# marcopesavento/Super-resolution-3D-Human-Shape-from-a-Single-Low-Resolution-Image

Measured on AMD Instinct MI355X. Metric: occupancy queries/sec (dense 512^3 reconstruction: encoder + query sweep + 2x marching cubes), higher is better.
Workload: dtype bf16

## Files before the change

super-resolution-3d-human-shape-from-a-single-low-resolution-image_amd/csrc/surs_api.cpp:

```cpp
#include "surs_common.h"

extern "C" int surs_abi_version(void) { return SURS_ABI_VERSION; }

extern "C" const char *surs_last_error(void) { return surs::err_buf(); }

extern "C" int surs_device_info(int *cu_count, char *arch_out) {
    int dev = 0;
    SURS_HIP_CHECK(hipGetDevice(&dev));
    hipDeviceProp_t prop;
    SURS_HIP_CHECK(hipGetDeviceProperties(&prop, dev));
    if (cu_count) *cu_count = prop.multiProcessorCount;
    if (arch_out) {
        strncpy(arch_out, prop.gcnArchName, 31);
        arch_out[31] = 0;
    }
    return 0;
}

#include <atomic>
#include <cstdlib>
#include <mutex>

namespace {
struct OptionRow {
    const char *name, *env;
    int def;
    char env_first;
    int env_value;
    const char *what;
};
const OptionRow kOptions[surs::OPT_COUNT] = {
    {"split_parts", "SURS_SPLIT", 2, 'b', 3, "operand parts of the fp32-grade GEMMs: 2 (f16 x 2) or 3 (bf16 x 3; env: bf16x3)"},
    {"grid_f32_columns", "SURS_GRID_F32", 1, 'g', 0, "0 (env: gemm): the fp32 sweep on the per-point layer kernels"},
    {"grid_kernel", "SURS_GRID_KERNEL", 0, 0, 0, "reduced-precision column kernel: 0 (default 12), 3, 10, 12"},
    {"grid_f32_kernel", "SURS_GRID_F32_KERNEL", 0, 0, 0, "fp32-grade column kernel: 0 (default 11), 5, 11"},
    {"r_parts", "SURS_R_PARTS", 1, 0, 0, "1: the bf16 sweep's R vectors from one f16 part; 0: the sweep's split"},
    {"grid_f32_passes", "SURS_GRID_F32_PASSES", 2, 0, 0, "passes of the fp32-grade column kernel per batch: 2 (lr, then hr) or 1"},
    {"bicubic_block", "SURS_BICUBIC_BLOCK", 1, 0, 0, "0: bicubic x2 with statistics one output per item (A/B; same bits)"},
    {"mc_emit_reclassify", "SURS_MC_EMIT_RECLASSIFY", 0, 0, 0, "1: marching cubes' emit pass classifies again (tests)"},
    {"point_runs_speculate", "SURS_POINT_RUNS_SPECULATE", 1, 0, 0, "0: surs_query_points_columns reads the run count before it launches"},
    {"conv_trace", "SURS_CONV_TRACE", 0, 0, 0, "diagnostic builds (-DSURS_CONV_TRACE): print the 3x3 kernel's phase stamps"},
    {"v3_trace", "SURS_V3_TRACE", 0, 0, 0, "diagnostic builds (-DSURS_V3_TRACE): print the column kernels' stamps"},
    {"conv_tall_min_wg", "SURS_CONV_TALL_MIN_WG", 256, 0, 0, "workgroups from which a stride-1 3x3 convolution takes the 8-row tile instead of 4 rows (0: never; same bits)"},
    {"conv_wide_min_wg", "SURS_CONV_WIDE_MIN_WG", 512, 0, 0, "workgroups (of 64 channels) from which such a launch takes 8 rows x 64 channels (part of the bits: another order of sums; 0: never)"},
    {"mc_ring", "SURS_MC_RING", 258, 0, 0, "planes of marching cubes' edge -> vertex-id ring = layers per chunk of a one-piece extraction + 1 (66: round 5's)"},
    {"rvec_small", "SURS_RVEC_SMALL", 1, 0, 0, "0: the affine part's GEMM of batches of <= 1024 columns on the 256 x 256-tile kernel (A/B; same bits)"},
    {"r_fused", "SURS_R_FUSED", 1, 0, 0, "0: the bf16 sweep's R vectors of batches of > 1024 columns from the g-scaled image and two GEMM launches (A/B; same bits)"},
};
std::atomic<int> g_option[surs::OPT_COUNT];
std::once_flag g_option_once;
void import_environment() {
    for (int i = 0; i < surs::OPT_COUNT; ++i) {
        const OptionRow &r = kOptions[i];
        int v = r.def;
        if (const char *e = getenv(r.env)) {
            if (r.env_first) v = (e[0] == r.env_first) ? r.env_value : r.def;
            else if (e[0]) v = atoi(e);
        }
        g_option[i].store(v, std::memory_order_relaxed);
    }
}
int find_option(const char *name) {
    if (!name) return -1;
    for (int i = 0; i < surs::OPT_COUNT; ++i)
        if (!strcmp(name, kOptions[i].name) || !strcmp(name, kOptions[i].env)) return i;
    return -1;
}
}

int surs::option(surs::Opt id) {
    std::call_once(g_option_once, import_environment);
    return g_option[id].load(std::memory_order_relaxed);
}

extern "C" int surs_set_option(const char *name, int value) {
    const int i = find_option(name);
    SURS_REQUIRE(i >= 0, "unknown option '%s' (surs_option_name(i) lists them)", name ? name : "(null)");
    std::call_once(g_option_once, import_environment);
    g_option[i].store(value, std::memory_order_relaxed);
    return 0;
// ... 12 lines not shown
```

super-resolution-3d-human-shape-from-a-single-low-resolution-image_amd/csrc/surs_common.h:

```cpp
#pragma once
#include <hip/hip_runtime.h>

#include <cstdarg>
#include <cstdio>
#include <cstring>

#include "../../include/surs.h"

namespace surs {

inline char *err_buf() {
    static thread_local char buf[512] = "";
    return buf;
}

inline int fail(int code, const char *fmt, ...) {
    va_list ap;
    va_start(ap, fmt);
    vsnprintf(err_buf(), 512, fmt, ap);
    va_end(ap);
    return code;
}

#define SURS_HIP_CHECK(expr)                                                                     \
    do {                                                                                         \
        hipError_t e_ = (expr);                                                                  \
        if (e_ != hipSuccess)                                                                    \
            return surs::fail(SURS_E_HIP, "%s:%d %s -> %s", __FILE__, __LINE__, #expr, hipGetErrorString(e_)); \
    } while (0)

#define SURS_LAUNCH_CHECK() SURS_HIP_CHECK(hipGetLastError())

#define SURS_REQUIRE(cond, ...)                                   \
    do {                                                          \
        if (!(cond)) return surs::fail(SURS_E_INVALID, __VA_ARGS__); \
    } while (0)

#ifndef SURS_ABL_NO_ISA_PINS
#define SURS_ISA_PIN(v) asm volatile("" : "+v"(v))
#else
#define SURS_ISA_PIN(v) do { } while (0)
#endif

enum Opt {
    OPT_SPLIT_PARTS, OPT_GRID_F32_COLUMNS, OPT_GRID_KERNEL, OPT_GRID_F32_KERNEL, OPT_R_PARTS,
    OPT_GRID_F32_PASSES, OPT_BICUBIC_BLOCK, OPT_MC_EMIT_RECLASSIFY, OPT_POINT_RUNS_SPECULATE, OPT_CONV_TRACE,
    OPT_V3_TRACE, OPT_CONV_TALL_MIN_WG, OPT_CONV_WIDE_MIN_WG, OPT_MC_RING, OPT_RVEC_SMALL, OPT_R_FUSED, OPT_COUNT
};
int option(Opt id);

inline hipStream_t as_stream(void *s) { return reinterpret_cast<hipStream_t>(s); }

constexpr int ceil_div(long long a, long long b) { return (int)((a + b - 1) / b); }

struct DeviceOnce {
    unsigned long long mask = 0;
    bool first() {
        int dev = 0;
        if (hipGetDevice(&dev) != hipSuccess || dev < 0 || dev >= 64) return true;
        const unsigned long long bit = 1ull << dev;
        const unsigned long long old = __atomic_fetch_or(&mask, bit, __ATOMIC_ACQ_REL);
        return !(old & bit);
    }
};
inline size_t align_up(size_t v, size_t a) { return (v + a - 1) / a * a; }

}
```

super-resolution-3d-human-shape-from-a-single-low-resolution-image_amd/csrc/surs_gemm.inc:

```
__device__ __forceinline__ bool gemm_block_tile(int mblocks, int nblocks, int &mb, int &nb) {
    const unsigned total = (unsigned)mblocks * (unsigned)nblocks, per = gridDim.x >> 3;
    const unsigned logical = (blockIdx.x & 7u) * per + (blockIdx.x >> 3);
    mb = (int)(logical % (unsigned)mblocks);
    nb = (int)(logical / (unsigned)mblocks);
    return logical < total;
}

static inline unsigned gemm_grid(int mblocks, long long nblocks) {
    const long long total = (long long)mblocks * nblocks;
    return (unsigned)(((total + 7) / 8) * 8);
}

struct SplitSeg {
    const unsigned short *base;
    long long part;
    int ktiles;
};

constexpr int G3_STAGES = 3;
constexpr int g3_stage_bytes(int bm, int np_ = 3) { return np_ * ((bm / 32) + 8) * 1024; }
constexpr int g3_lds_bytes(int bm, int np_ = 3) { return G3_STAGES * g3_stage_bytes(bm, np_); }

template <int NP> struct SplitKind;
template <> struct SplitKind<1> {
// ... 158 lines not shown
        } else
            asm volatile("s_waitcnt vmcnt(0)\n\ts_barrier" ::: "memory");
#endif
    };
    if (((wave >> 2) & 1) == 0) {
        for (int kt = 0; kt < ktiles; ++kt) {
            step_barrier(kt);
            phase1(kt);
            phase2(kt);
        }
    } else {
        step_barrier(0);
        phase1(0);
        for (int kt = 1; kt < ktiles; ++kt) {
            step_barrier(kt);
            phase2(kt - 1);
            phase1(kt);
        }
        phase2(ktiles - 1);
    }

#undef G3_RD
#undef G3_WAIT4
#undef G3_WAIT2
#pragma unroll
    for (int i = 0; i < TI; ++i)
#pragma unroll
        for (int j = 0; j < 2; ++j) {
            const long long n = n0 + wn * 64 + j * 32 + li;
            const int mrow = m0 + wm * (TI * 32) + i * 32;
            if constexpr (OUT == G3_F32_T) {
                const long long nb0 = n0 + wn * 64 + j * 32 + 4 * kh;
                const float bm = bias[mrow + li];
#pragma unroll
                for (int g = 0; g < 4; ++g)
#pragma unroll
                    for (int r = 0; r < 4; ++r) Y[(nb0 + 8 * g + r) * ldy + mrow + li] = acc[i][j][4 * g + r] + bm;
                continue;
            }
            float v[16];
#pragma unroll
            for (int g = 0; g < 4; ++g)
#pragma unroll
                for (int r = 0; r < 4; ++r) {
                    float t = acc[i][j][4 * g + r] + bias[mrow + 8 * g + 4 * kh + r];
                    v[4 * g + r] = t > 0.0f ? t : 0.01f * t;
                }
            if constexpr (OUT == G3_F32) {
#pragma unroll
                for (int g = 0; g < 4; ++g)
#pragma unroll
                    for (int r = 0; r < 4; ++r) Y[(long long)(mrow + 8 * g + 4 * kh + r) * ldy + n] = v[4 * g + r];
            } else
#pragma unroll
            for (int q = 0; q < 2; ++q) {
                unsigned e[NP][2], o[NP][2];
#pragma unroll
                for (int d = 0; d < 2; ++d) {
                    unsigned short x0[NP], x1[NP], y0[NP], y1[NP];
                    SK::split(v[8 * q + 2 * d], x0);
                    SK::split(v[8 * q + 2 * d + 1], x1);
                    SK::split(v[8 * q + 4 + 2 * d], y0);
                    SK::split(v[8 * q + 4 + 2 * d + 1], y1);
#pragma unroll
                    for (int p = 0; p < NP; ++p) {
                        e[p][d] = (unsigned)x0[p] | ((unsigned)x1[p] << 16);
                        o[p][d] = (unsigned)y0[p] | ((unsigned)y1[p] << 16);
                    }
                }
                unsigned short *dst = Ys + ((long long)((mrow >> 4) + q) * np + n) * 16 + kh * 8;
// ... 202 lines not shown
                const vec8 w = wf[t];
#pragma unroll
                for (int j = 0; j < NT; ++j) acc[j] = SK::mfma(x[t & 1][j], w, acc[j]);
                if (t < NQ) {
                    f32x4 wz, wp;
                    zload(sf, wz, wp);
                    form(t, ring[t], wz, wp, smem + (u ^ 1) * RVF_STAGE_BYTES);
                    ring[t] = load(sl, t);
                }
                wf[t] = wload(kt + PF < KT ? kt + PF : KT - 1);
            }
            __syncthreads();
#pragma unroll
            for (int j = 0; j < NT; ++j) x[0][j] = *reinterpret_cast<const vec8 *>(rd + (u ^ 1) * RVF_STAGE_BYTES + j * PS);
        }
    }
    float *out = a.r[M] + (size_t)col0 * NV * D2 + m0 + li;
#pragma unroll
    for (int j = 0; j < NT; ++j)
#pragma unroll
        for (int gq = 0; gq < 4; ++gq)
#pragma unroll
            for (int r = 0; r < 4; ++r) out[(size_t)(32 * j + 4 * kh + 8 * gq + r) * D2] = acc[j][4 * gq + r] + 0.0f;
}

__global__ __launch_bounds__(RVF_THREADS) void rvec_fused_kernel(RvecFusedArgs a) {
    extern __shared__ __attribute__((aligned(16))) unsigned char rvf_smem[];
    int mb, nb;
    if (!gemm_block_tile(D2 / RVF_ROWS, a.tiles, mb, nb)) return;
    const int col0 = nb * RVF_COLS, m0 = mb * RVF_ROWS + (int)(threadIdx.x >> 6) * 32;
    rvec_fused_phase<0>(a, rvf_smem, col0, m0);
    rvec_fused_phase<1>(a, rvf_smem, col0, m0);
}
```

super-resolution-3d-human-shape-from-a-single-low-resolution-image_amd/csrc/surs_query.hip:

```cpp
#include <hip/hip_runtime.h>

#include <cstdlib>
#include <map>
#include <mutex>
#include <type_traits>
#include <utility>
#include <vector>

#include "surs_common.h"
#include "surs_mlp_generic.h"
#include "surs_mlp_layout.h"

namespace surs {

typedef float f32x16 __attribute__((ext_vector_type(16)));
typedef float f32x4 __attribute__((ext_vector_type(4)));
typedef unsigned u32x4 __attribute__((ext_vector_type(4)));
typedef unsigned u32x2 __attribute__((ext_vector_type(2)));
typedef float f32x2 __attribute__((ext_vector_type(2)));

struct PointSource {
    int mode;
    const float *pts;
    const long long *idx;
// ... 68 lines not shown
    pix[3] = (long long)cy1 * W + cx1;
}

__device__ __forceinline__ float tap_sum(const float (&t)[4], const float (&w)[4]) {
    float a = 0.0f;
    a += t[0] * w[0];
    a += t[1] * w[1];
    a += t[2] * w[2];
    a += t[3] * w[3];
    return a;
}

typedef __bf16 bf16x8_t __attribute__((ext_vector_type(8)));
typedef unsigned short u16x8_t __attribute__((ext_vector_type(8)));

__device__ __forceinline__ void split3_bf16(float x, unsigned short &a, unsigned short &b, unsigned short &c) {
    const __bf16 ha = (__bf16)x;
    const float r1 = x - (float)ha;
    const __bf16 hb = (__bf16)r1;
    const float r2 = r1 - (float)hb;
    const __bf16 hc = (__bf16)r2;
    a = __builtin_bit_cast(unsigned short, ha);
    b = __builtin_bit_cast(unsigned short, hb);
    c = __builtin_bit_cast(unsigned short, hc);
}

#include "surs_gemm.inc"

template <int NP>
__global__ __launch_bounds__(256) void gather_kernel(PointSource src, long long n, const float *__restrict__ feat_lr,
                                                     int hl, int wl, const float *__restrict__ feat_hr, int hh,
                                                     int wh, float *__restrict__ F, long long ldf,
                                                     float *__restrict__ mask, float *__restrict__ zproj,
                                                     unsigned short *__restrict__ Fs, long long fs_part) {
    __shared__ float tile[64][65];
    __shared__ float sx[64], sy[64];
    const int tid = threadIdx.x, lane = tid & 63, wave = tid >> 6;
    const long long n0 = (long long)blockIdx.x * 64;
    const bool lead = blockIdx.y == 0;
    if (tid < 64) {
        long long t = n0 + tid;
        float X = 2.0f, Y = 2.0f;
        if (t < n) {
            float px, py, pz;
            make_point(src, t, px, py, pz);
            float Z;
            project_point(src, px, py, pz, X, Y, Z);
            const float in = in_image(X, Y);
            if (lead) {
                mask[t] = in;
                if (zproj) zproj[t] = Z;
                F[(long long)C_G * ldf + t] = Z * src.zmul / src.zdiv;
                F[(long long)(C_G + 1) * ldf + t] = 0.0f;
            }
            if (Fs && lead) {
                unsigned short zp[NP];
                SplitKind<NP>::split(Z * src.zmul / src.zdiv, zp);
#pragma unroll
                for (int p = 0; p < NP; ++p) {
                    u16x8_t v = {zp[p], 0, 0, 0, 0, 0, 0, 0}, z = {0, 0, 0, 0, 0, 0, 0, 0};
                    u16x8_t *dst = reinterpret_cast<u16x8_t *>(Fs + p * fs_part + ((long long)(C_G / 16) * ldf + t) * 16);
                    dst[0] = v;
                    dst[1] = z;
                }
            }
        }
        sx[tid] = X;
        sy[tid] = Y;
    }
    __syncthreads();
    for (int chunk = blockIdx.y; chunk < 5; chunk += gridDim.y) {
        const bool is_hr = chunk == 4;
// ... 171 lines not shown
}

static int g_split_override = 0;
static thread_local int t_split_call = 0;
static int split_parts() {
    const int v = option(OPT_SPLIT_PARTS) == 3 ? 3 : 2;
    return t_split_call > 1 ? t_split_call : (g_split_override ? g_split_override : v);
}

template <int NP, int... More, class F> static void with_parts(int parts, F &&f) {
    if constexpr (sizeof...(More) == 0) f(std::integral_constant<int, NP>());
    else if (parts == NP) f(std::integral_constant<int, NP>());
    else with_parts<More...>(parts, f);
}

static int g3_set_attributes() {
    static DeviceOnce attr;
    if (attr.first()) {
        SURS_HIP_CHECK(hipFuncSetAttribute((const void *)gemm_x3g_kernel<8, 256, G3_SPLIT, 2>, hipFuncAttributeMaxDynamicSharedMemorySize, g3_lds_bytes(256, 2)));
        SURS_HIP_CHECK(hipFuncSetAttribute((const void *)gemm_x3g_kernel<8, 256, G3_F32, 2>, hipFuncAttributeMaxDynamicSharedMemorySize, g3_lds_bytes(256, 2)));
        SURS_HIP_CHECK(hipFuncSetAttribute((const void *)gemm_x3g_kernel<8, 128, G3_F32, 2>, hipFuncAttributeMaxDynamicSharedMemorySize, g3_lds_bytes(128, 2)));
        SURS_HIP_CHECK(hipFuncSetAttribute((const void *)gemm_x3g_kernel<8, 128, G3_F32_T, 2>, hipFuncAttributeMaxDynamicSharedMemorySize, g3_lds_bytes(128, 2)));
        SURS_HIP_CHECK(hipFuncSetAttribute((const void *)gemm_x3g_kernel<8, 256, G3_SPLIT>, hipFuncAttributeMaxDynamicSharedMemorySize, g3_lds_bytes(256)));
        SURS_HIP_CHECK(hipFuncSetAttribute((const void *)gemm_x3g_kernel<8, 256, G3_F32>, hipFuncAttributeMaxDynamicSharedMemorySize, g3_lds_bytes(256)));
        SURS_HIP_CHECK(hipFuncSetAttribute((const void *)gemm_x3g_kernel<8, 128, G3_F32>, hipFuncAttributeMaxDynamicSharedMemorySize, g3_lds_bytes(128)));
        SURS_HIP_CHECK(hipFuncSetAttribute((const void *)gemm_x3g_kernel<8, 128, G3_F32_T>, hipFuncAttributeMaxDynamicSharedMemorySize, g3_lds_bytes(128)));
        SURS_HIP_CHECK(hipFuncSetAttribute((const void *)gemm_x3g_kernel<8, 256, G3_F32_T, 2>, hipFuncAttributeMaxDynamicSharedMemorySize, g3_lds_bytes(256, 2)));
        SURS_HIP_CHECK(hipFuncSetAttribute((const void *)gemm_x3g_kernel<8, 256, G3_F32_T>, hipFuncAttributeMaxDynamicSharedMemorySize, g3_lds_bytes(256)));
        SURS_HIP_CHECK(hipFuncSetAttribute((const void *)gemm_x3g_kernel<8, 256, G3_F32_T, 1>, hipFuncAttributeMaxDynamicSharedMemorySize, g3_lds_bytes(256, 1)));
        SURS_HIP_CHECK(hipFuncSetAttribute((const void *)gemm_x3g_kernel<8, 256, G3_SPLIT, 1>, hipFuncAttributeMaxDynamicSharedMemorySize, g3_lds_bytes(256, 1)));
        SURS_HIP_CHECK(hipFuncSetAttribute((const void *)gemm_x3g_kernel<8, 256, G3_F32, 1>, hipFuncAttributeMaxDynamicSharedMemorySize, g3_lds_bytes(256, 1)));
        SURS_HIP_CHECK(hipFuncSetAttribute((const void *)gemm_x3g_kernel<8, 128, G3_F32, 1>, hipFuncAttributeMaxDynamicSharedMemorySize, g3_lds_bytes(128, 1)));
        SURS_HIP_CHECK(hipFuncSetAttribute((const void *)rvec_fused_kernel, hipFuncAttributeMaxDynamicSharedMemorySize, RVF_LDS_BYTES));
    }
    return 0;
}

static int launch_layer(hipStream_t st, int parts, int out, const void *W, int M, SplitSeg s1, SplitSeg s2, long long np, long long n,
                        const float *bias, float *Y, unsigned short *Ys) {
    SURS_REQUIRE(parts >= 1 && parts <= 3, "layer kernel: 1, 2 or 3 operand parts");
    SURS_REQUIRE(np % 256 == 0 && n % 256 == 0 && n <= np, "the layer kernel needs 256-point tiles");
    SURS_REQUIRE(M % 256 == 0 || (out != G3_SPLIT && M % 128 == 0), "layer kernel rows: a multiple of 256 (of 128 for an fp32 output)");
    SURS_REQUIRE(M % 256 == 0 || out != G3_F32_T || parts > 1, "no one-part layer kernel for a transposed output of 128-row tiles");
    int rc = g3_set_attributes();
    if (rc) return rc;
    const int K = 16 * (s1.ktiles + s2.ktiles), nb = (int)(n / 256);
    const long long ldy = out == G3_F32_T ? M : np;
    with_parts<1, 2, 3>(parts, [&](auto NP) {
        auto go = [&](auto BM, auto OUT) {
            hipLaunchKernelGGL((gemm_x3g_kernel<8, BM, OUT, NP>), dim3(gemm_grid(M / BM, nb)), dim3(512), g3_lds_bytes(BM, NP), st,
                               (const unsigned short *)W, M, K, s1, s2, np, bias, Y, ldy, Ys, (long long)M * np, nb);
        };
        using C256 = std::integral_constant<int, 256>;
        using C128 = std::integral_constant<int, 128>;
        if (out == G3_SPLIT) go(C256(), std::integral_constant<int, G3_SPLIT>());
        else if (out == G3_F32) {
            if (M % 256 == 0) go(C256(), std::integral_constant<int, G3_F32>());
            else go(C128(), std::integral_constant<int, G3_F32>());
        } else if (M % 256 == 0) go(C256(), std::integral_constant<int, G3_F32_T>());
        else if constexpr (NP > 1) go(C128(), std::integral_constant<int, G3_F32_T>());
    });
    SURS_LAUNCH_CHECK();
    return 0;
}

static int run_points_fp32(hipStream_t st, const PointSource &src, long long n, const float *feat_lr, int hl, int wl,
                           const float *feat_hr, int hh, int wh, const char *blob, const MlpBlobHeader &h,
                           const Fp32Workspace &w, float *pred_hr, float *pred_lr, float *logit_hr, float *logit_lr,
                           int parts = 0, const float *p_lr_in = nullptr, bool lr_only = false) {
    const long long np = w.np;
    if (parts == 0) parts = t_split_call == 1 ? 1 : split_parts();
    const long long fs_part = (long long)C0PAD * np;
    with_parts<1, 2, 3>(parts, [&](auto NP) {
        hipLaunchKernelGGL(gather_kernel<NP>, dim3((unsigned)ceil_div(n, 64)), dim3(256), 0, st, src, n, feat_lr, hl, wl, feat_hr,
                           hh, wh, w.F, np, w.mask, (float *)nullptr, w.Fs, fs_part);
    });
    SURS_LAUNCH_CHECK();
    if (p_lr_in) {
        with_parts<1, 2, 3>(parts, [&](auto NP) {
            hipLaunchKernelGGL(patch_plr_kernel<NP>, dim3((unsigned)ceil_div(n, 256)), dim3(256), 0, st, p_lr_in, np, n,
                               w.F + (size_t)(C_G + 1) * np, w.Fs, fs_part);
        });
        SURS_LAUNCH_CHECK();
    }
    const SplitSeg none = {nullptr, 0, 0}, f = {w.Fs, fs_part, C0PAD / 16}, y0 = {w.Y0s, (long long)D1 * np, D1 / 16},
                   y1 = {w.Y1s, (long long)D2 * np, D2 / 16}, y2 = {w.Y2s, (long long)D3 * np, D3 / 16};
    for (int m = p_lr_in ? 1 : 0; m < (lr_only ? 1 : 2); ++m) {
        auto W = [&](int l) { return (const void *)(blob + (parts <= 2 ? h.wt2[m][l] : h.wt3[m][l])); };
        auto BI = [&](int l) { return (const float *)(blob + h.bias[m][l]); };
        int rc;
        if ((rc = launch_layer(st, parts, G3_SPLIT, W(0), D1, f, none, np, np, BI(0), nullptr, w.Y0s))) return rc;
        if ((rc = launch_layer(st, parts, G3_SPLIT, W(1), D2, y0, none, np, np, BI(1), nullptr, w.Y1s))) return rc;
        if ((rc = launch_layer(st, parts, G3_SPLIT, W(2), D3, y1, f, np, np, BI(2), nullptr, w.Y2s))) return rc;
        if ((rc = launch_layer(st, parts, G3_F32, W(3), D4, y2, f, np, np, BI(3), w.Y3, nullptr))) return rc;
        with_parts<1, 2, 3>(parts, [&](auto NP) {
            hipLaunchKernelGGL(mlp_last_kernel<NP>, dim3((unsigned)ceil_div(n, 256)), dim3(256), 0, st,
                               (const float *)(blob + h.w4[m]), w.Y3, w.F, np, n, w.mask, m == 0 ? pred_lr : pred_hr,
                               m == 0 ? logit_lr : logit_hr, m == 0 ? w.F + (size_t)(C_G + 1) * np : (float *)nullptr,
                               m == 0 ? w.Fs : (unsigned short *)nullptr, fs_part);
        });
        SURS_LAUNCH_CHECK();
    }
    return 0;
}

template <int DT> struct HalfT;
template <> struct HalfT<SURS_BF16> {
    typedef __bf16 elem;
// ... 238 lines not shown
    return views_ws_bytes((long long)ceil_div(max_points, 256) * 256, num_views < 1 ? 1 : num_views);
}

static int run_points_views(hipStream_t st, const PointSource *srcs, int n, int num_views, const float *feat_lr, int hl, int wl,
                            const float *feat_hr, int hh, int wh, const void *mlp_blob, void *workspace, float *pred_hr, float *pred_lr,
                            float *logit_hr, float *logit_lr) {
    const long long np = (long long)ceil_div(n, 256) * 256;
    const MlpBlobHeader h = blob_layout(SURS_BF16);
    const char *blob = (const char *)mlp_blob;
    const int V = num_views;
    float *p = (float *)workspace;
    float *F = p;      p += (size_t)V * C0PAD * np;
    float *Y2 = p;     p += (size_t)V * D3 * np;
    float *mask = p;   p += (size_t)V * np;
    p += (size_t)(D1 + D2) * np;
    float *Y3 = p;     p += (size_t)D4 * np;
    float *Fm = p;     p += (size_t)C0PAD * np;
    float *Y2m = p;    p += (size_t)D3 * np;
    const long long fstride = (long long)C0PAD * np;
    const int parts = split_parts();
    unsigned short *q = (unsigned short *)p;
    unsigned short *Fs = q;   q += (size_t)V * 3 * fstride;
    unsigned short *Y0s = q;  q += (size_t)3 * D1 * np;
    unsigned short *Y1s = q;  q += (size_t)3 * D2 * np;
    unsigned short *Y2ms = q; q += (size_t)3 * D3 * np;
    unsigned short *Fms = q;
    for (int v = 0; v < V; ++v) {
        float *Fv = F + (size_t)v * fstride;
        SURS_HIP_CHECK(hipMemsetAsync(Fv + (size_t)(C_G + 2) * np, 0, (size_t)(C0PAD - C_G - 2) * np * sizeof(float), st));
        const PointSource &src = srcs[v];
        with_parts<2, 3>(parts, [&](auto NP) {
            hipLaunchKernelGGL(gather_kernel<NP>, dim3((unsigned)ceil_div(n, 64)), dim3(256), 0, st, src, (long long)n,
                               feat_lr + (size_t)v * hl * wl * C_LR, hl, wl, feat_hr + (size_t)v * hh * wh * C_HR, hh, wh, Fv, np,
                               mask + (size_t)v * np, (float *)nullptr, Fs + (size_t)v * parts * fstride, fstride);
        });
        SURS_LAUNCH_CHECK();
    }
    const SplitSeg none = {nullptr, 0, 0}, y0 = {Y0s, (long long)D1 * np, D1 / 16}, y1 = {Y1s, (long long)D2 * np, D2 / 16},
                   y2m = {Y2ms, (long long)D3 * np, D3 / 16}, fm = {Fms, fstride, C0PAD / 16};
    for (int m = 0; m < 2; ++m) {
        auto W = [&](int l) { return (const void *)(blob + (parts == 2 ? h.wt2[m][l] : h.wt3[m][l])); };
        auto BI = [&](int l) { return (const float *)(blob + h.bias[m][l]); };
        int rc;
        for (int v = 0; v < V; ++v) {
            const SplitSeg fv = {Fs + (size_t)v * parts * fstride, fstride, C0PAD / 16};
            if ((rc = launch_layer(st, parts, G3_SPLIT, W(0), D1, fv, none, np, np, BI(0), nullptr, Y0s))) return rc;
            if ((rc = launch_layer(st, parts, G3_SPLIT, W(1), D2, y0, none, np, np, BI(1), nullptr, Y1s))) return rc;
            if ((rc = launch_layer(st, parts, G3_F32, W(2), D3, y1, fv, np, np, BI(2), Y2 + (size_t)v * D3 * np, nullptr))) return rc;
        }
        const float inv = 1.0f / (float)V;
        hipLaunchKernelGGL(mean_views_kernel, dim3((unsigned)ceil_div((long long)D3 * np, 256)), dim3(256), 0, st, Y2,
                           (long long)D3 * np, V, (long long)D3 * np, inv, Y2m);
        SURS_LAUNCH_CHECK();
        hipLaunchKernelGGL(mean_views_kernel, dim3((unsigned)ceil_div(fstride, 256)), dim3(256), 0, st, F, fstride, V, fstride,
                           inv, Fm);
        SURS_LAUNCH_CHECK();
        with_parts<2, 3>(parts, [&](auto NP) {
            hipLaunchKernelGGL(split_rows_kernel<NP>, dim3((unsigned)ceil_div(np, 256), D3 / 16), dim3(256), 0, st, Y2m, np, D3 / 16,
                               Y2ms, (long long)D3 * np);
            hipLaunchKernelGGL(split_rows_kernel<NP>, dim3((unsigned)ceil_div(np, 256), C0PAD / 16), dim3(256), 0, st, Fm, np,
                               C0PAD / 16, Fms, fstride);
        });
        SURS_LAUNCH_CHECK();
        if ((rc = launch_layer(st, parts, G3_F32, W(3), D4, y2m, fm, np, np, BI(3), Y3, nullptr))) return rc;
        with_parts<2, 3>(parts, [&](auto NP) {
            hipLaunchKernelGGL(mlp_last_views_kernel<NP>, dim3((unsigned)ceil_div(n, 256)), dim3(256), 0, st,
                               (const float *)(blob + h.w4[m]), Y3, Fm, np, (long long)n, V, mask, m == 0 ? pred_lr : pred_hr,
// ... 143 lines not shown
}
static size_t col_v7_image_bytes(long long ncb) { return (size_t)ncb * 5 * D1 * 6; }
static size_t col_v7_bytes(long long ncb) { return col_v7_image_bytes(ncb) + (size_t)ncb * 5 * D2 * 4 + D2 * 4 + 256; }
static size_t col_ws_bytes(long long ncb) { return col_base_bytes(ncb) + col_v7_bytes(ncb); }

extern "C" size_t surs_query_grid_workspace_bytes(int ry, int rz, int dtype) {
    (void)ry; (void)rz;
    const size_t col = col_ws_bytes(COL_BATCH);
    if (dtype == SURS_F32 || dtype == SURS_F32_GEMM) {
        const size_t gen = fp32_ws_bytes(GRID_BATCH);
        return gen > col ? gen : col;
    }
    return col;
}

static bool grid_f32_use_columns() { return option(OPT_GRID_F32_COLUMNS) != 0; }

static int grid_set_attributes() {
    static DeviceOnce attr;
    if (!attr.first()) return 0;
    SURS_HIP_CHECK(hipFuncSetAttribute((const void *)grid_mlp_kernel_v3<SURS_BF16>, hipFuncAttributeMaxDynamicSharedMemorySize, GRID3_LDS_BYTES));
    SURS_HIP_CHECK(hipFuncSetAttribute((const void *)grid_mlp_kernel_v3<SURS_F16>, hipFuncAttributeMaxDynamicSharedMemorySize, GRID3_LDS_BYTES));
    SURS_HIP_CHECK(hipFuncSetAttribute((const void *)grid_mlp_kernel_v5, hipFuncAttributeMaxDynamicSharedMemorySize, GRID5_LDS_BYTES));
    SURS_HIP_CHECK(hipFuncSetAttribute((const void *)grid_mlp_kernel_v11, hipFuncAttributeMaxDynamicSharedMemorySize, GRID11_LDS_BYTES));
    SURS_HIP_CHECK(hipFuncSetAttribute((const void *)grid_mlp_kernel_v10<SURS_BF16>, hipFuncAttributeMaxDynamicSharedMemorySize, GRID10_LDS_BYTES));
    SURS_HIP_CHECK(hipFuncSetAttribute((const void *)grid_mlp_kernel_v10<SURS_F16>, hipFuncAttributeMaxDynamicSharedMemorySize, GRID10_LDS_BYTES));
    SURS_HIP_CHECK(hipFuncSetAttribute((const void *)grid_mlp_kernel_v12<SURS_BF16>, hipFuncAttributeMaxDynamicSharedMemorySize, GRID12_LDS_BYTES));
    SURS_HIP_CHECK(hipFuncSetAttribute((const void *)grid_mlp_kernel_v12<SURS_F16>, hipFuncAttributeMaxDynamicSharedMemorySize, GRID12_LDS_BYTES));
    return 0;
}

static int column_constants(hipStream_t st, const PointSource &src, long long nc, long long ncp, const float *feat_lr, int hl, int wl,
                            const float *feat_hr, int hh, int wh, const char *blob, const MlpBlobHeader &h, float *F, float *CC,
                            float *cmask) {
    const int parts = split_parts();
    unsigned short *Fs = (unsigned short *)(cmask + COL_BATCH);
    const long long fs_part = (long long)C0PAD * COL_BATCH;
    const dim3 gg((unsigned)ceil_div(nc, 64), nc <= 4096 ? 5u : 1u);
    with_parts<2, 3>(parts, [&](auto NP) {
        hipLaunchKernelGGL(gather_kernel<NP>, gg, dim3(256), 0, st, src, nc, feat_lr, hl, wl, feat_hr, hh, wh, F, COL_BATCH, cmask,
                           (float *)nullptr, Fs, fs_part);
    });
    SURS_LAUNCH_CHECK();
    const SplitSeg f = {Fs, fs_part, C_G / 16}, none = {nullptr, 0, 0};
    return launch_layer(st, parts, G3_F32_T, blob + (parts == 2 ? h.wc2 : h.wc3), CC_PAD, f, none, COL_BATCH, ncp,
                        (const float *)(blob + h.bc), CC, nullptr);
}

__global__ __launch_bounds__(256) void probe_count_kernel(const float *__restrict__ cc, const float *__restrict__ zvec, int rz, int tile,
                                                          double z0, double dz, float c22, float c23, float zmul, float zdiv, float zmid,
                                                          unsigned long long *__restrict__ out) {
    const int tid = threadIdx.x;
    const float *row = cc + (size_t)blockIdx.x * CC_PAD;
    const f32x4 al = *reinterpret_cast<const f32x4 *>(row + CC_A0_LR + 4 * tid), ah = *reinterpret_cast<const f32x4 *>(row + CC_A0_HR + 4 * tid);
    const f32x4 zl = *reinterpret_cast<const f32x4 *>(zvec + ZV_W0Z_LR + 4 * tid), zh = *reinterpret_cast<const f32x4 *>(zvec + ZV_W0Z_HR + 4 * tid);
    const f32x4 ph = *reinterpret_cast<const f32x4 *>(zvec + ZV_W0P_HR + 4 * tid);
    auto zf_of = [&](int k) {
        const double zt = dz * (double)k;
        const float zw = (float)(zt + z0);
        const float Z = c23 + c22 * zw;
        return Z * zmul / zdiv;
    };
    unsigned nl = 0, nh = 0;
    for (int k0 = 0; k0 < rz; k0 += tile) {
        const float e0 = zf_of(k0), e1 = zf_of(k0 + tile - 1);
        const float zlo = fminf(e0, e1), zhi = fmaxf(e0, e1);
#pragma unroll
        for (int i = 0; i < 4; ++i) {
            {
                const float xm = fmaf(zmid, zl[i], al[i]);
                const float t0 = zl[i] * zlo, t1 = zl[i] * zhi;
                const float mn = al[i] + fminf(t0, t1), mx = al[i] + fmaxf(t0, t1);
                nl += ((xm > 0.0f) ? (mn > 0.0f) : (mx <= 0.0f)) ? 0u : 1u;
            }
// ... 74 lines not shown
    const int ve = option(OPT_GRID_KERNEL), ve32 = option(OPT_GRID_F32_KERNEL);
    const int kver_env = (ve == 3 || ve == 10 || ve == 12) ? ve : SURS_DEFAULT_GRID_KERNEL;
    const int kver32_env = (ve32 == 5 || ve32 == 11) ? ve32 : SURS_DEFAULT_GRID_F32_KERNEL;
    const auto is32 = [](int v) { return v == 5 || v == 11; };
    kver = kver_env;
    kver32 = kver32_env;
    if (g_grid_kernel_override) (is32(g_grid_kernel_override) ? kver32 : kver) = g_grid_kernel_override;
    if (kernel_call) (is32(kernel_call) ? kver32 : kver) = kernel_call;
}

static int device_cus() {
    int dev = 0;
    hipDeviceProp_t prop;
    if (hipGetDevice(&dev) == hipSuccess && hipGetDeviceProperties(&prop, dev) == hipSuccess) return prop.multiProcessorCount;
    return 256;
}

static int run_column_batch(const ColumnSweep &cs, const PointSource &src, long long nc, int items, int zstride,
                            const int *kcount, const unsigned short *klist, float *vol_hr, float *vol_lr, bool trace_this) {
    hipStream_t st = cs.st;
    const char *blob = cs.blob;
    const MlpBlobHeader &h = cs.h;
    const int dtype = cs.dtype, kver = cs.kver, kver32 = cs.kver32;
    const bool restated = cs.restated;
    const double *mat = cs.mat;
    const float *calib = cs.calib;
    void *workspace = cs.workspace;
    float *F = (float *)workspace;
    float *CC = F + (size_t)C0PAD * COL_BATCH;
    float *cmask = CC + (size_t)CC_PAD * COL_BATCH;
    int rc = 0;
    const long long ncp = (long long)ceil_div(nc, 256) * 256;
    const int parts = split_parts();
    if ((rc = column_constants(st, src, nc, ncp, cs.feat_lr, cs.hl, cs.wl, cs.feat_hr, cs.hh, cs.wh, blob, h, F, CC, cmask))) return rc;
    GridArgs a;
    a.cc = CC;
    a.colmask = cmask;
    a.zvec = (const float *)(blob + h.zvec);
    a.core = blob + h.core;
    a.corex = blob + h.corex;
    a.b1frag = blob + h.b1frag;
    a.b1_inv_scale = 1.0f / (dtype == SURS_F16 ? B1FRAG_SCALE_F16 : B1FRAG_SCALE_BF16);
    a.w1t = blob + h.w1t;
    a.w1tx = blob + h.w1tx;
    a.rvec_lr = a.rvec_hr = nullptr;
    a.rld_lr = a.rld_hr = 0;
    a.colctr = nullptr;
    a.phase = 0;
    a.zmid = 0.0f;
    a.zstride = zstride;
    a.kcount = kcount;
    a.klist = klist;
    a.ovf_count = nullptr;
    a.ovf_list = nullptr;
    a.aimg = nullptr;
    a.tile_list = cs.run_tiles;
    a.tile_count = cs.run_ntiles;
    a.colstart = cs.run_colstart;
    a.zpts = cs.run_z;
    if (restated) {
        char *v7 = (char *)workspace + col_base_bytes(COL_BATCH);
        unsigned short *g_lr = (unsigned short *)v7, *g_hr = g_lr + (size_t)COL_BATCH * 2 * D1 * 3;
        float *r_lr = (float *)(v7 + col_v7_image_bytes(COL_BATCH)), *r_hr = r_lr + (size_t)COL_BATCH * 2 * D2;
        float *zero_bias = r_hr + (size_t)COL_BATCH * 3 * D2;
        a.colctr = (unsigned *)(zero_bias + D2);
        {
            const float zw = cs.run_z ? 0.0f : (float)(mat[10] * (double)cs.kmid + mat[11]);
            a.zmid = (calib[11] + calib[10] * zw) * cs.zmul / cs.zdiv;
        }
        const long long part_lr = 2LL * ncp * D1, part_hr = 3LL * ncp * D1;
        const dim3 pg((unsigned)(ncp / 4));
        const int r_parts_env = option(OPT_R_PARTS);
        const int rparts = (dtype == SURS_BF16 && r_parts_env == 1) ? 1 : parts;
        const bool fused = rparts == 1 && ncp > 1024 && option(OPT_R_FUSED);
        if (fused) SURS_HIP_CHECK(hipMemsetAsync(a.colctr, 0, 256, st));
        else SURS_HIP_CHECK(hipMemsetAsync(zero_bias, 0, D2 * 4 + 256, st));
        if (!fused) {
            with_parts<1, 2, 3>(rparts, [&](auto NP) {
                hipLaunchKernelGGL(colsum_prepare_kernel<NP>, pg, dim3(256), 0, st, CC, (const float *)(blob + h.zvec), (int)ncp, a.zmid,
                                   g_lr, part_lr, g_hr, part_hr);
            });
            SURS_LAUNCH_CHECK();
        }
        if (fused) {
            RvecFusedArgs fa;
            fa.cc = CC;
            fa.zvec = (const float *)(blob + h.zvec);
            fa.zmid = a.zmid;
            fa.tiles = (int)(ncp / RVF_COLS);
            for (int m = 0; m < 2; ++m) {
                fa.w[m] = (const unsigned short *)(blob + h.wt2[m][1]);
                fa.r[m] = m ? r_hr : r_lr;
            }
            if ((rc = g3_set_attributes())) return rc;
            hipLaunchKernelGGL(rvec_fused_kernel, dim3(gemm_grid(D2 / RVF_ROWS, fa.tiles)), dim3(RVF_THREADS), RVF_LDS_BYTES, st, fa);
            SURS_LAUNCH_CHECK();
        } else if (ncp <= 1024 && option(OPT_RVEC_SMALL)) {
            RvecSmallArgs ra;
            for (int m = 0; m < 2; ++m) {
                const int nvec = m ? 3 : 2;
                ra.w[m] = (const unsigned short *)(blob + (rparts == 3 ? h.wt3[m][1] : h.wt2[m][1]));
                ra.g[m] = m ? g_hr : g_lr;
                ra.g_part[m] = m ? part_hr : part_lr;
                ra.npm[m] = (long long)nvec * ncp;
                ra.r[m] = m ? r_hr : r_lr;
            }
            ra.wgs0 = (int)(ra.npm[0] / 64) * 4;
            const unsigned wgs = (unsigned)(ra.wgs0 + (ra.npm[1] / 64) * 4);
            with_parts<1, 2, 3>(rparts, [&](auto NP) { hipLaunchKernelGGL(rvec_small_kernel<NP>, dim3(wgs), dim3(256), 0, st, ra); });
            SURS_LAUNCH_CHECK();
        } else {
            const SplitSeg none = {nullptr, 0, 0};
            for (int m = 0; m < 2; ++m) {
                const long long npm = (m ? 3LL : 2LL) * ncp;
                const SplitSeg g = {m ? g_hr : g_lr, m ? part_hr : part_lr, D1 / 16};
                if ((rc = launch_layer(st, rparts, G3_F32_T, blob + (rparts == 3 ? h.wt3[m][1] : h.wt2[m][1]), D2, g, none, npm, npm,
                                       zero_bias, m ? r_hr : r_lr, nullptr)))
                    return rc;
            }
        }
        a.rvec_lr = r_lr;
        a.rvec_hr = r_hr;
        a.rld_lr = a.rld_hr = 0;
    }
    a.vol_hr = vol_hr;
    a.vol_lr = vol_lr;
    a.ncols = (int)nc;
    a.rz = items;
// ... 775 lines not shown
```

Before: 1.197 billion.

## Add warp-specialized R-vector kernel with loader waves feeding MFMA waves

```diff
diff --git a/super-resolution-3d-human-shape-from-a-single-low-resolution-image_amd/csrc/surs_api.cpp b/super-resolution-3d-human-shape-from-a-single-low-resolution-image_amd/csrc/surs_api.cpp
--- a/super-resolution-3d-human-shape-from-a-single-low-resolution-image_amd/csrc/surs_api.cpp
+++ b/super-resolution-3d-human-shape-from-a-single-low-resolution-image_amd/csrc/surs_api.cpp
@@ -46,6 +46,7 @@
     {"mc_ring", "SURS_MC_RING", 258, 0, 0, "planes of marching cubes' edge -> vertex-id ring = layers per chunk of a one-piece extraction + 1 (66: round 5's)"},
     {"rvec_small", "SURS_RVEC_SMALL", 1, 0, 0, "0: the affine part's GEMM of batches of <= 1024 columns on the 256 x 256-tile kernel (A/B; same bits)"},
     {"r_fused", "SURS_R_FUSED", 1, 0, 0, "0: the bf16 sweep's R vectors of batches of > 1024 columns from the g-scaled image and two GEMM launches (A/B; same bits)"},
+    {"r_loader", "SURS_R_LOADER", 1, 0, 0, "0: those batches' one R kernel with every wave loading, forming and multiplying (rvec_fused_kernel) instead of loader waves beside multiplier waves (A/B; same bits)"},
 };
 std::atomic<int> g_option[surs::OPT_COUNT];
 std::once_flag g_option_once;
diff --git a/super-resolution-3d-human-shape-from-a-single-low-resolution-image_amd/csrc/surs_common.h b/super-resolution-3d-human-shape-from-a-single-low-resolution-image_amd/csrc/surs_common.h
--- a/super-resolution-3d-human-shape-from-a-single-low-resolution-image_amd/csrc/surs_common.h
+++ b/super-resolution-3d-human-shape-from-a-single-low-resolution-image_amd/csrc/surs_common.h
@@ -45,7 +45,7 @@
 enum Opt {
     OPT_SPLIT_PARTS, OPT_GRID_F32_COLUMNS, OPT_GRID_KERNEL, OPT_GRID_F32_KERNEL, OPT_R_PARTS,
     OPT_GRID_F32_PASSES, OPT_BICUBIC_BLOCK, OPT_MC_EMIT_RECLASSIFY, OPT_POINT_RUNS_SPECULATE, OPT_CONV_TRACE,
-    OPT_V3_TRACE, OPT_CONV_TALL_MIN_WG, OPT_CONV_WIDE_MIN_WG, OPT_MC_RING, OPT_RVEC_SMALL, OPT_R_FUSED, OPT_COUNT
+    OPT_V3_TRACE, OPT_CONV_TALL_MIN_WG, OPT_CONV_WIDE_MIN_WG, OPT_MC_RING, OPT_RVEC_SMALL, OPT_R_FUSED, OPT_R_LOADER, OPT_COUNT
 };
 int option(Opt id);
 
diff --git a/super-resolution-3d-human-shape-from-a-single-low-resolution-image_amd/csrc/surs_gemm.inc b/super-resolution-3d-human-shape-from-a-single-low-resolution-image_amd/csrc/surs_gemm.inc
--- a/super-resolution-3d-human-shape-from-a-single-low-resolution-image_amd/csrc/surs_gemm.inc
+++ b/super-resolution-3d-human-shape-from-a-single-low-resolution-image_amd/csrc/surs_gemm.inc
@@ -214,10 +214,16 @@
             if constexpr (OUT == G3_F32_T) {
                 const long long nb0 = n0 + wn * 64 + j * 32 + 4 * kh;
                 const float bm = bias[mrow + li];
+#ifdef SURS_G3_NO_T_STORES
+#ifdef __HIP_DEVICE_COMPILE__
+                asm volatile("" ::"v"(acc[i][j]), "v"(bm), "v"((int)nb0));
+#endif
+#else
 #pragma unroll
                 for (int g = 0; g < 4; ++g)
 #pragma unroll
                     for (int r = 0; r < 4; ++r) Y[(nb0 + 8 * g + r) * ldy + mrow + li] = acc[i][j][4 * g + r] + bm;
+#endif
                 continue;
             }
             float v[16];
@@ -486,3 +492,256 @@
     rvec_fused_phase<0>(a, rvf_smem, col0, m0);
     rvec_fused_phase<1>(a, rvf_smem, col0, m0);
 }
+
+constexpr int RVL_MWAVES = 8, RVL_LWAVES = 8, RVL_LTHREADS = 64 * RVL_LWAVES, RVL_THREADS = 64 * RVL_MWAVES + RVL_LTHREADS;
+constexpr int RVL_KS = 4;
+constexpr int RVL_RING = 4;
+constexpr int RVL_X_BYTES = RVL_KS * 6 * RVF_PIECE;
+constexpr int RVL_WT_BYTES = (RVF_ROWS / 32) * 1024;
+constexpr int RVL_W_BYTES = RVL_KS * RVL_WT_BYTES;
+constexpr int RVL_STAGE_BYTES = RVL_X_BYTES + RVL_W_BYTES;
+constexpr int RVL_STEPS = D1 / (16 * RVL_KS);
+constexpr int RVL_LDS_BYTES = 2 * RVL_STAGE_BYTES + 3 * D1 * 4;
+constexpr int RVL_CG = RVL_LTHREADS / 16, RVL_NQ = RVF_COLS / RVL_CG;
+constexpr int RVL_NW = RVL_W_BYTES / (RVL_LTHREADS * 16);
+static_assert(RVL_CG == 32 && RVL_THREADS == 1024, "a pass of the loaders = 32 columns = NV whole point tiles; sixteen waves, 128 registers");
+static_assert(RVL_STEPS % RVL_RING == 0 && RVL_RING % 2 == 0 && RVL_X_BYTES % 16 == 0 && RVL_LDS_BYTES <= 160 * 1024, "a0 ring of four steps; 160 KB of LDS");
+
+#define RVL_BARRIER() asm volatile("s_waitcnt lgkmcnt(0)\n\ts_barrier" ::: "memory")
+
+struct RvlWalk {
+    unsigned first, end, stride;
+};
+
+template <int M>
+__device__ __forceinline__ void rvl_multiply_phase(const RvecFusedArgs &a, const unsigned char *smem, int wave, int lane, int col0, int row0, bool more) {
+    typedef SplitKind<1> SK;
+    typedef SK::vec8 vec8;
+    constexpr int NV = M ? 3 : 2, NT = 2 * NV, KS = RVL_KS, PS = RVF_PIECE;
+    const int kh = lane >> 5, li = lane & 31, rg = wave >> 1, ph = wave & 1;
+    const unsigned char *xrd = smem + ph * NV * PS + kh * RVF_HALF + li * 16;
+    const unsigned char *wrd = smem + RVL_X_BYTES + 2 * rg * 1024 + lane * 16;
+    f32x16 acc[2][NV];
+#pragma unroll
+    for (int i = 0; i < 2; ++i)
+#pragma unroll
+        for (int j = 0; j < NV; ++j)
+#pragma unroll
+            for (int q = 0; q < 16; ++q) acc[i][j][q] = 0.0f;
+    vec8 x[NV], w[2];
+    auto read = [&](int t, const unsigned char *xs, const unsigned char *ws) {
+#pragma unroll
+        for (int i = 0; i < 2; ++i) w[i] = *reinterpret_cast<const vec8 *>(ws + t * RVL_WT_BYTES + i * 1024);
+#pragma unroll
+        for (int j = 0; j < NV; ++j) x[j] = *reinterpret_cast<const vec8 *>(xs + (t * NT + j) * PS);
+    };
+#pragma unroll 1
+    for (int s2 = 0; s2 < RVL_STEPS; s2 += 2) {
+#pragma unroll
+        for (int u = 0; u < 2; ++u) {
+            if (s2 + u) RVL_BARRIER();
+            const unsigned char *xs = xrd + u * RVL_STAGE_BYTES, *ws = wrd + u * RVL_STAGE_BYTES;
+            read(0, xs, ws);
+#pragma unroll
+            for (int t = 0; t < KS; ++t) {
+                __builtin_amdgcn_sched_barrier(0);
+#pragma unroll
+                for (int i = 0; i < 2; ++i)
+#pragma unroll
+                    for (int j = 0; j < NV; ++j) acc[i][j] = SK::mfma(x[j], w[i], acc[i][j]);
+                if (t + 1 < KS) {
+                    __builtin_amdgcn_sched_barrier(0);
+                    read(t + 1, xs, ws);
+                }
+            }
+        }
+    }
+    if (more) RVL_BARRIER();
+#ifndef SURS_RVL_NO_STORES
+    int ln = 0;
+    asm volatile("" : "+v"(ln));
+    ln = (int)__builtin_amdgcn_mbcnt_hi(~0u, __builtin_amdgcn_mbcnt_lo(~0u, (unsigned)ln));
+    const int odd = ln & 1;
+    float *out = a.r[M] + ((size_t)col0 * NV + 32 * NV * ph + 4 * (ln >> 5) + odd) * D2 + row0 + 64 * rg + (ln & 31) - odd;
+#pragma unroll
+    for (int i = 0; i < 2; ++i)
+#pragma unroll
+        for (int j = 0; j < NV; ++j)
+#pragma unroll
+            for (int gq = 0; gq < 4; ++gq)
+#pragma unroll
+                for (int r = 0; r < 4; r += 2) {
+                    const float va = acc[i][j][4 * gq + r] + 0.0f, vb = acc[i][j][4 * gq + r + 1] + 0.0f;
+                    const float send = odd ? va : vb;
+                    const float recv = __builtin_bit_cast(float, __builtin_amdgcn_update_dpp(0, __builtin_bit_cast(int, send), 0xB1, 0xF, 0xF, false));
+                    const f32x2 v = {odd ? recv : va, odd ? vb : recv};
+                    *reinterpret_cast<f32x2 *>(out + (size_t)(32 * j + 8 * gq + r) * D2 + 32 * i) = v;
+                }
+#else
+#pragma unroll
+    for (int i = 0; i < 2; ++i)
+#pragma unroll
+        for (int j = 0; j < NV; ++j) asm volatile("" ::"v"(acc[i][j]));
+#endif
+}
+
+__device__ __forceinline__ void rvl_multiply(const RvecFusedArgs &a, const unsigned char *smem, int wave, int lane, RvlWalk wk) {
+#ifdef SURS_RVL_MULT_PRIO
+    __builtin_amdgcn_s_setprio(SURS_RVL_MULT_PRIO);
+#endif
+    RVL_BARRIER();
+    RVL_BARRIER();
+    for (unsigned logical = wk.first; logical < wk.end; logical += wk.stride) {
+        const int col0 = (int)(logical >> 1) * RVF_COLS, row0 = (int)(logical & 1u) * RVF_ROWS;
+        rvl_multiply_phase<0>(a, smem, wave, lane, col0, row0, true);
+        rvl_multiply_phase<1>(a, smem, wave, lane, col0, row0, logical + wk.stride < wk.end);
+    }
+}
+
+struct RvlSrc {
+    unsigned a0;
+    unsigned w;
+};
+
+__device__ __forceinline__ f32x4 rvl_a0(const RvecFusedArgs &a, unsigned off) {
+    return *reinterpret_cast<const f32x4 *>(reinterpret_cast<const char *>(a.cc) + off);
+}
+__device__ __forceinline__ u32x4 rvl_w(const unsigned short *w, unsigned off, int h) {
+    return *reinterpret_cast<const u32x4 *>(reinterpret_cast<const char *>(w) + (off + (unsigned)((h * RVL_LTHREADS * 16 / RVL_WT_BYTES) * (D2 * 32) + (h * RVL_LTHREADS * 16) % RVL_WT_BYTES)));
+}
+
+template <int M>
+__device__ __forceinline__ void rvl_load_phase(const RvecFusedArgs &a, unsigned char *smem, int lt, RvlSrc cur, RvlSrc nxt, f32x4 (&ring)[RVL_RING][RVL_NQ], u32x4 (&wr)[RVL_NW]) {
+    typedef SplitKind<1> SK;
+    typedef _Float16 f16x2 __attribute__((ext_vector_type(2)));
+    constexpr int NV = M ? 3 : 2, NT = 2 * NV, KS = RVL_KS, NQ = RVL_NQ, PS = RVF_PIECE;
+    const int fc = lt >> 4, fq = lt & 15;
+    const float zmid = a.zmid;
+    const float *zs = reinterpret_cast<const float *>(smem + 2 * RVL_STAGE_BYTES) + (M ? D1 : 0) + 4 * fq;
+    unsigned char *xw[NV];
+#pragma unroll
+    for (int v = 0; v < NV; ++v) {
+            const int p = fc * NV + v;
+            xw[v] = smem + (unsigned)(((fq >> 2) * NT * PS) + (((fq & 3) >> 1) * RVF_HALF) + (fq & 1) * 8 + (p >> 5) * PS + (p & 31) * 16);
+        }
+    auto form = [&](int q, const f32x4 a0, const f32x4 wz, const f32x4 wp, int stage) {
+        float val[NV][4];
+#pragma unroll
+        for (int e = 0; e < 4; ++e) {
+            float g;
+            if constexpr (M) {
+                g = fmaf(0.5f, wp[e], fmaf(zmid, wz[e], a0[e])) > 0.0f ? 1.0f : 0.01f;
+                val[NV - 1][e] = g * wp[e];
+            } else {
+                g = fmaf(zmid, wz[e], a0[e]) > 0.0f ? 1.0f : 0.01f;
+            }
+            val[0][e] = g * a0[e];
+            val[1][e] = g * wz[e];
+        }
+#pragma unroll
+        for (int v = 0; v < NV; ++v) {
+            unsigned pr[2];
+#pragma unroll
+            for (int d = 0; d < 2; ++d) {
+                unsigned short p0[1], p1[1];
+#ifdef SURS_RVL_NO_FORM
+                p0[0] = (unsigned short)__builtin_bit_cast(unsigned, a0[2 * d]);
+                p1[0] = (unsigned short)__builtin_bit_cast(unsigned, a0[2 * d + 1]);
+#else
+                SK::split(val[v][2 * d], p0);
+                SK::split(val[v][2 * d + 1], p1);
+#endif
+                const f16x2 h = {__builtin_bit_cast(_Float16, p0[0]), __builtin_bit_cast(_Float16, p1[0])};
+                pr[d] = __builtin_bit_cast(unsigned, h);
+            }
+            *reinterpret_cast<u32x2 *>(xw[v] + (stage * RVL_STAGE_BYTES + q * NV * PS)) = u32x2{pr[0], pr[1]};
+        }
+    };
+    unsigned char *ww = smem + RVL_X_BYTES + lt * 16;
+#pragma unroll 1
+    for (int s4 = 0; s4 < RVL_STEPS; s4 += RVL_RING) {
+        const bool wrap = s4 + RVL_RING == RVL_STEPS;
+        const unsigned la = (wrap ? nxt.a0 : cur.a0) + 64 * KS * (wrap ? 0 : s4 + RVL_RING);
+#pragma unroll
+        for (int u = 0; u < RVL_RING; ++u) {
+            const int s = s4 + u;
+            f32x4 wz = *reinterpret_cast<const f32x4 *>(zs + 16 * KS * s), wp = wz;
+            if constexpr (M) wp = *reinterpret_cast<const f32x4 *>(zs + D1 + 16 * KS * s);
+#pragma unroll
+            for (int q = 0; q < NQ; ++q) form(q, ring[u][q], wz, wp, u & 1);
+#pragma unroll
+            for (int h = 0; h < RVL_NW; ++h) *reinterpret_cast<u32x4 *>(ww + ((u & 1) * RVL_STAGE_BYTES + h * RVL_LTHREADS * 16)) = wr[h];
+            __builtin_amdgcn_sched_barrier(0);
+            const bool wrapw = u == RVL_RING - 1 && wrap;
+            const unsigned short *lwb = wrapw ? a.w[M ^ 1] : a.w[M];
+            const unsigned lw = wrapw ? nxt.w : cur.w + (unsigned)(s + 1) * (KS * D2 * 32);
+#pragma unroll
+            for (int h = 0; h < RVL_NW; ++h) wr[h] = rvl_w(lwb, lw, h);
+            __builtin_amdgcn_sched_barrier(0);
+#ifndef SURS_RVL_NO_A0
+#pragma unroll
+            for (int q = 0; q < NQ; ++q) ring[u][q] = rvl_a0(a, la + (unsigned)(RVL_CG * q * CC_PAD * 4 + 64 * KS * u));
+#endif
+            RVL_BARRIER();
+        }
+    }
+}
+
+__device__ __forceinline__ void rvl_load(const RvecFusedArgs &a, unsigned char *smem, int lt, RvlWalk wk) {
+    constexpr int NQ = RVL_NQ;
+    const int fc = lt >> 4, fq = lt & 15;
+#ifdef SURS_RVL_LOADER_PRIO
+    __builtin_amdgcn_s_setprio(SURS_RVL_LOADER_PRIO);
+#endif
+    {
+        float *zs = reinterpret_cast<float *>(smem + 2 * RVL_STAGE_BYTES);
+        for (int i = lt; i < 3 * D1 / 4; i += RVL_LTHREADS) {
+            const int v = i >> 8, c = 4 * (i & 255);
+            *reinterpret_cast<f32x4 *>(zs + v * D1 + c) = *reinterpret_cast<const f32x4 *>(a.zvec + (v == 0 ? ZV_W0Z_LR : v == 1 ? ZV_W0Z_HR : ZV_W0P_HR) + c);
+        }
+    }
+    auto src = [&](unsigned logical, int m) {
+        RvlSrc s;
+        s.a0 = 4u * (((logical >> 1) * RVF_COLS + fc) * (unsigned)CC_PAD + (unsigned)((m ? CC_A0_HR : CC_A0_LR) + 4 * fq));
+        s.w = (logical & 1u) * RVL_WT_BYTES + lt * 16;
+        return s;
+    };
+    unsigned logical = wk.first;
+    RvlSrc lr = src(logical, 0), hr = src(logical, 1);
+    f32x4 ring[RVL_RING][NQ];
+    u32x4 wr[RVL_NW];
+#pragma unroll
+    for (int h = 0; h < RVL_NW; ++h) wr[h] = rvl_w(a.w[0], lr.w, h);
+#pragma unroll
+    for (int u = 0; u < RVL_RING; ++u)
+#pragma unroll
+        for (int q = 0; q < NQ; ++q) ring[u][q] = rvl_a0(a, lr.a0 + (unsigned)(RVL_CG * q * CC_PAD * 4 + 64 * RVL_KS * u));
+    RVL_BARRIER();
+    for (;;) {
+        const unsigned next = logical + wk.stride;
+        const bool more = next < wk.end;
+        const RvlSrc nlr = src(more ? next : logical, 0);
+        rvl_load_phase<0>(a, smem, lt, lr, hr, ring, wr);
+        rvl_load_phase<1>(a, smem, lt, hr, nlr, ring, wr);
+        if (!more) break;
+        logical = next;
+        lr = nlr;
+        hr = src(logical, 1);
+    }
+}
+
+__global__ __launch_bounds__(RVL_THREADS) void rvec_loader_kernel(RvecFusedArgs a) {
+    extern __shared__ __attribute__((aligned(16))) unsigned char rvl_smem[];
+    RvlWalk wk;
+    {
+        const unsigned total = 2u * (unsigned)a.tiles, per = (total + 7u) >> 3, xcd = blockIdx.x & 7u, slot = blockIdx.x >> 3;
+        wk.first = xcd * per + slot;
+        wk.end = (xcd + 1u) * per < total ? (xcd + 1u) * per : total;
+        wk.stride = gridDim.x >> 3;
+        if (slot >= per || wk.first >= wk.end) return;
+    }
+    const int wave = __builtin_amdgcn_readfirstlane((int)(threadIdx.x >> 6));
+    if (wave < RVL_MWAVES) rvl_multiply(a, rvl_smem, wave, (int)(threadIdx.x & 63), wk);
+    else rvl_load(a, rvl_smem, (int)threadIdx.x - RVL_MWAVES * 64, wk);
+}
+#undef RVL_BARRIER
diff --git a/super-resolution-3d-human-shape-from-a-single-low-resolution-image_amd/csrc/surs_query.hip b/super-resolution-3d-human-shape-from-a-single-low-resolution-image_amd/csrc/surs_query.hip
--- a/super-resolution-3d-human-shape-from-a-single-low-resolution-image_amd/csrc/surs_query.hip
+++ b/super-resolution-3d-human-shape-from-a-single-low-resolution-image_amd/csrc/surs_query.hip
@@ -124,12 +124,14 @@
                                                      int hl, int wl, const float *__restrict__ feat_hr, int hh,
                                                      int wh, float *__restrict__ F, long long ldf,
                                                      float *__restrict__ mask, float *__restrict__ zproj,
-                                                     unsigned short *__restrict__ Fs, long long fs_part) {
+                                                     unsigned short *__restrict__ Fs, long long fs_part,
+                                                     unsigned *__restrict__ ctr) {
     __shared__ float tile[64][65];
     __shared__ float sx[64], sy[64];
     const int tid = threadIdx.x, lane = tid & 63, wave = tid >> 6;
     const long long n0 = (long long)blockIdx.x * 64;
     const bool lead = blockIdx.y == 0;
+    if (ctr && blockIdx.x == 0 && lead && tid >= 64 && tid < 128) ctr[tid - 64] = 0u;
     if (tid < 64) {
         long long t = n0 + tid;
         float X = 2.0f, Y = 2.0f;
@@ -367,6 +369,7 @@
         SURS_HIP_CHECK(hipFuncSetAttribute((const void *)gemm_x3g_kernel<8, 256, G3_F32, 1>, hipFuncAttributeMaxDynamicSharedMemorySize, g3_lds_bytes(256, 1)));
         SURS_HIP_CHECK(hipFuncSetAttribute((const void *)gemm_x3g_kernel<8, 128, G3_F32, 1>, hipFuncAttributeMaxDynamicSharedMemorySize, g3_lds_bytes(128, 1)));
         SURS_HIP_CHECK(hipFuncSetAttribute((const void *)rvec_fused_kernel, hipFuncAttributeMaxDynamicSharedMemorySize, RVF_LDS_BYTES));
+        SURS_HIP_CHECK(hipFuncSetAttribute((const void *)rvec_loader_kernel, hipFuncAttributeMaxDynamicSharedMemorySize, RVL_LDS_BYTES));
     }
     return 0;
 }
@@ -408,7 +411,7 @@
     const long long fs_part = (long long)C0PAD * np;
     with_parts<1, 2, 3>(parts, [&](auto NP) {
         hipLaunchKernelGGL(gather_kernel<NP>, dim3((unsigned)ceil_div(n, 64)), dim3(256), 0, st, src, n, feat_lr, hl, wl, feat_hr,
-                           hh, wh, w.F, np, w.mask, (float *)nullptr, w.Fs, fs_part);
+                           hh, wh, w.F, np, w.mask, (float *)nullptr, w.Fs, fs_part, (unsigned *)nullptr);
     });
     SURS_LAUNCH_CHECK();
     if (p_lr_in) {
@@ -713,7 +716,7 @@
         with_parts<2, 3>(parts, [&](auto NP) {
             hipLaunchKernelGGL(gather_kernel<NP>, dim3((unsigned)ceil_div(n, 64)), dim3(256), 0, st, src, (long long)n,
                                feat_lr + (size_t)v * hl * wl * C_LR, hl, wl, feat_hr + (size_t)v * hh * wh * C_HR, hh, wh, Fv, np,
-                               mask + (size_t)v * np, (float *)nullptr, Fs + (size_t)v * parts * fstride, fstride);
+                               mask + (size_t)v * np, (float *)nullptr, Fs + (size_t)v * parts * fstride, fstride, (unsigned *)nullptr);
         });
         SURS_LAUNCH_CHECK();
     }
@@ -923,14 +926,14 @@
 
 static int column_constants(hipStream_t st, const PointSource &src, long long nc, long long ncp, const float *feat_lr, int hl, int wl,
                             const float *feat_hr, int hh, int wh, const char *blob, const MlpBlobHeader &h, float *F, float *CC,
-                            float *cmask) {
+                            float *cmask, unsigned *ctr = nullptr) {
     const int parts = split_parts();
     unsigned short *Fs = (unsigned short *)(cmask + COL_BATCH);
     const long long fs_part = (long long)C0PAD * COL_BATCH;
     const dim3 gg((unsigned)ceil_div(nc, 64), nc <= 4096 ? 5u : 1u);
     with_parts<2, 3>(parts, [&](auto NP) {
         hipLaunchKernelGGL(gather_kernel<NP>, gg, dim3(256), 0, st, src, nc, feat_lr, hl, wl, feat_hr, hh, wh, F, COL_BATCH, cmask,
-                           (float *)nullptr, Fs, fs_part);
+                           (float *)nullptr, Fs, fs_part, ctr);
     });
     SURS_LAUNCH_CHECK();
     const SplitSeg f = {Fs, fs_part, C_G / 16}, none = {nullptr, 0, 0};
@@ -1071,7 +1074,13 @@
     int rc = 0;
     const long long ncp = (long long)ceil_div(nc, 256) * 256;
     const int parts = split_parts();
-    if ((rc = column_constants(st, src, nc, ncp, cs.feat_lr, cs.hl, cs.wl, cs.feat_hr, cs.hh, cs.wh, blob, h, F, CC, cmask))) return rc;
+    const int rparts = (dtype == SURS_BF16 && option(OPT_R_PARTS) == 1) ? 1 : parts;
+    const bool fused = restated && rparts == 1 && ncp > 1024 && option(OPT_R_FUSED);
+    float *const zero_bias =
+        restated ? (float *)((char *)workspace + col_base_bytes(COL_BATCH) + col_v7_image_bytes(COL_BATCH)) + (size_t)COL_BATCH * 5 * D2 : nullptr;
+    if ((rc = column_constants(st, src, nc, ncp, cs.feat_lr, cs.hl, cs.wl, cs.feat_hr, cs.hh, cs.wh, blob, h, F, CC, cmask,
+                               fused ? (unsigned *)(zero_bias + D2) : nullptr)))
+        return rc;
     GridArgs a;
     a.cc = CC;
     a.colmask = cmask;
@@ -1101,7 +1110,6 @@
         char *v7 = (char *)workspace + col_base_bytes(COL_BATCH);
         unsigned short *g_lr = (unsigned short *)v7, *g_hr = g_lr + (size_t)COL_BATCH * 2 * D1 * 3;
         float *r_lr = (float *)(v7 + col_v7_image_bytes(COL_BATCH)), *r_hr = r_lr + (size_t)COL_BATCH * 2 * D2;
-        float *zero_bias = r_hr + (size_t)COL_BATCH * 3 * D2;
         a.colctr = (unsigned *)(zero_bias + D2);
         {
             const float zw = cs.run_z ? 0.0f : (float)(mat[10] * (double)cs.kmid + mat[11]);
@@ -1109,11 +1117,7 @@
         }
         const long long part_lr = 2LL * ncp * D1, part_hr = 3LL * ncp * D1;
         const dim3 pg((unsigned)(ncp / 4));
-        const int r_parts_env = option(OPT_R_PARTS);
-        const int rparts = (dtype == SURS_BF16 && r_parts_env == 1) ? 1 : parts;
-        const bool fused = rparts == 1 && ncp > 1024 && option(OPT_R_FUSED);
-        if (fused) SURS_HIP_CHECK(hipMemsetAsync(a.colctr, 0, 256, st));
-        else SURS_HIP_CHECK(hipMemsetAsync(zero_bias, 0, D2 * 4 + 256, st));
+        if (!fused) SURS_HIP_CHECK(hipMemsetAsync(zero_bias, 0, D2 * 4 + 256, st));
         if (!fused) {
             with_parts<1, 2, 3>(rparts, [&](auto NP) {
                 hipLaunchKernelGGL(colsum_prepare_kernel<NP>, pg, dim3(256), 0, st, CC, (const float *)(blob + h.zvec), (int)ncp, a.zmid,
@@ -1132,7 +1136,11 @@
                 fa.r[m] = m ? r_hr : r_lr;
             }
             if ((rc = g3_set_attributes())) return rc;
-            hipLaunchKernelGGL(rvec_fused_kernel, dim3(gemm_grid(D2 / RVF_ROWS, fa.tiles)), dim3(RVF_THREADS), RVF_LDS_BYTES, st, fa);
+            if (option(OPT_R_LOADER)) {
+                const unsigned items_grid = gemm_grid(D2 / RVF_ROWS, fa.tiles), cu_grid = (unsigned)(cs.cus > 8 ? cs.cus & ~7 : 8);
+                hipLaunchKernelGGL(rvec_loader_kernel, dim3(items_grid < cu_grid ? items_grid : cu_grid), dim3(RVL_THREADS), RVL_LDS_BYTES, st, fa);
+            } else
+                hipLaunchKernelGGL(rvec_fused_kernel, dim3(gemm_grid(D2 / RVF_ROWS, fa.tiles)), dim3(RVF_THREADS), RVF_LDS_BYTES, st, fa);
             SURS_LAUNCH_CHECK();
         } else if (ncp <= 1024 && option(OPT_RVEC_SMALL)) {
             RvecSmallArgs ra;
```

After: 1.199 billion (median of 2 runs). No clear change (+0.2%).
